# artiom-matvei/RLAO

Measured on AMD Instinct MI355X. Metric: AO env-steps/sec (batched loops), higher is better.
Workload: dtype f32; 1 GPU; 8m / 20x20 Shack-Hartmann, 256 batched envs per GPU, integrator closed loop (BASELINE.json configs[1]); envs_per_gpu=256, envs_total=256, resolution=120, n_valid_act=357, n_signal=632, layers=1, controller=leaky integrator, gain 0.5, noise=photon, parallelism=env-shards x1, all-gather of episode returns

## Files before the change

rlao_amd/csrc/ring_device.hpp:

```cpp
#pragma once
#include "common.hpp"

namespace ao {

__device__ inline int torus(int r, int c, int oy, int ox, int S) {
    int pr = r + oy, pc = c + ox;
    pr = pr >= S ? pr - S : pr;
    pc = pc >= S ? pc - S : pc;
    return pr * S + pc;
}

template <typename T>
__device__ inline void gather_ring(const T* __restrict__ map, T* __restrict__ zx, const int* __restrict__ inner_idx, int S,
                                   int n_inner, int K, int sx, int sy, int oy, int ox, int e, int t0, int nt) {
    const T* src = map + (size_t)e * S * S;
    for (int k = t0; k < n_inner; k += nt) {
        const int idx = inner_idx[k];
        const int r = idx / S - sy, c = idx % S - sx;
        zx[(size_t)e * K + k] = src[torus(r, c, oy, ox, S)];
    }
}

__device__ inline uint32_t mt_temper(uint32_t y) {
    y ^= (y >> 11);
    y ^= (y << 7) & 0x9d2c5680u;
    y ^= (y << 15) & 0xefc60000u;
    y ^= (y >> 18);
    return y;
}

__device__ inline uint32_t mt_mix(uint32_t a, uint32_t b, uint32_t far) {
    uint32_t y = (a & 0x80000000u) | (b & 0x7fffffffu);
    return far ^ (y >> 1) ^ ((y & 1u) ? 0x9908b0dfu : 0u);
}

__device__ inline void mt_twist(uint32_t* s) {
    const int t = threadIdx.x;
    uint32_t v = 0;
    if (t < 227) v = mt_mix(s[t], s[t + 1], s[t + 397]);
    __syncthreads();
    if (t < 227) s[t] = v;
    __syncthreads();
    if (t < 227) v = mt_mix(s[t + 227], s[t + 228], s[t]);
    __syncthreads();
    if (t < 227) s[t + 227] = v;
    __syncthreads();
    if (t < 169) v = mt_mix(s[t + 454], s[t + 455], s[t + 227]);
    __syncthreads();
    if (t < 169) s[t + 454] = v;
    __syncthreads();
    if (t == 0) s[623] = mt_mix(s[623], s[0], s[396]);
    __syncthreads();
}

template <typename T>
__device__ inline void mt_normal_body(const uint32_t* mt_state, const int* mt_pos, uint32_t* mt_state_out, int* mt_pos_out,
                                      T* __restrict__ zx, int K, int n_inner, int n_outer, int e, const double* xi_scale) {
    __shared__ uint32_t s[kMtN];
    __shared__ int scan[256];
    __shared__ int sh_pos, sh_got, sh_stop;
    const int t = threadIdx.x;
    const uint32_t* gs = mt_state + (size_t)e * kMtN;
    uint32_t* gso = mt_state_out + (size_t)e * kMtN;
    for (int i = t; i < kMtN; i += 256) s[i] = gs[i];
    if (t == 0) {
        sh_pos = mt_pos[e];
        sh_got = 0;
    }
    __syncthreads();
    const int need_pairs = n_outer / 2;
    T* out = zx + (size_t)e * K + n_inner;
    while (true) {
        if (sh_pos >= kMtN) {
            mt_twist(s);
            if (t == 0) sh_pos = 0;
            __syncthreads();
        }
        const int pos = sh_pos, got = sh_got;
        const int avail = (kMtN - pos) / 4;
        int acc = 0;
        double n0 = 0.0, n1 = 0.0;
        if (t < avail) {
            const uint32_t* w = s + pos + 4 * t;
            const double d1 = ((double)(mt_temper(w[0]) >> 5) * 67108864.0 + (double)(mt_temper(w[1]) >> 6)) /
                              9007199254740992.0;
            const double d2 = ((double)(mt_temper(w[2]) >> 5) * 67108864.0 + (double)(mt_temper(w[3]) >> 6)) /
                              9007199254740992.0;
            const double x1 = 2.0 * d1 - 1.0, x2 = 2.0 * d2 - 1.0;
            const double r2 = x1 * x1 + x2 * x2;
            if (r2 < 1.0 && r2 != 0.0) {
                acc = 1;
                const double f = sqrt(-2.0 * log(r2) / r2);
                n0 = f * x2;
                n1 = f * x1;
                if (xi_scale) {
                    const double sg = xi_scale[e];
                    n0 *= sg;
                    n1 *= sg;
                }
            }
        }
        const unsigned long long bal = __ballot(acc);
        const int lane = t & (kWave - 1), wv = t / kWave;
        const int in_wave = __popcll(bal & ((lane == 63) ? ~0ull : ((2ull << lane) - 1ull)));
        if (lane == 0) scan[wv] = __popcll(bal);
        __syncthreads();
        int before = 0;
        for (int q = 0; q < wv; ++q) before += scan[q];
        const int total_acc = scan[0] + scan[1] + scan[2] + scan[3];
        const int incl = before + in_wave;
        const int remaining = need_pairs - got;
        if (t == 0) sh_stop = -1;
        __syncthreads();
        if (acc && incl <= remaining) {
            const int j = got + incl - 1;
            out[2 * j] = (T)n0;
            out[2 * j + 1] = (T)n1;
            if (incl == remaining) sh_stop = t;
        }
        __syncthreads();
        if (sh_stop >= 0) {
            if (t == 0) sh_pos = pos + 4 * (sh_stop + 1);
            break;
        }
        if (t == 0) {
            sh_pos = kMtN;
            sh_got = got + total_acc;
        }
        __syncthreads();
    }
    __syncthreads();
    for (int i = t; i < kMtN; i += 256) gso[i] = s[i];
    if (t == 0) mt_pos_out[e] = sh_pos;
}

}
```

Measured before the change: 5.653 million env-steps/s.

## Batch multiple Mersenne Twister twists per round and process two polar pairs per thread

```diff
diff --git a/rlao_amd/csrc/ring_device.hpp b/rlao_amd/csrc/ring_device.hpp
--- a/rlao_amd/csrc/ring_device.hpp
+++ b/rlao_amd/csrc/ring_device.hpp
@@ -34,104 +34,116 @@
     return far ^ (y >> 1) ^ ((y & 1u) ? 0x9908b0dfu : 0u);
 }
 
-__device__ inline void mt_twist(uint32_t* s) {
+constexpr int kMtTry = kMtN / 4;
+constexpr int kMtSlots = 4;
+constexpr int kMtLaneTry = 2 * 256;
+
+__device__ inline void mt_twist_next(const uint32_t* s, uint32_t* n) {
     const int t = threadIdx.x;
-    uint32_t v = 0;
-    if (t < 227) v = mt_mix(s[t], s[t + 1], s[t + 397]);
+    if (t < 227) n[t] = mt_mix(s[t], s[t + 1], s[t + 397]);
     __syncthreads();
-    if (t < 227) s[t] = v;
+    if (t < 227) n[t + 227] = mt_mix(s[t + 227], s[t + 228], n[t]);
     __syncthreads();
-    if (t < 227) v = mt_mix(s[t + 227], s[t + 228], s[t]);
+    if (t < 169) n[t + 454] = mt_mix(s[t + 454], s[t + 455], n[t + 227]);
+    if (t == 192) n[623] = mt_mix(s[623], n[0], n[396]);
     __syncthreads();
-    if (t < 227) s[t + 227] = v;
-    __syncthreads();
-    if (t < 169) v = mt_mix(s[t + 454], s[t + 455], s[t + 227]);
-    __syncthreads();
-    if (t < 169) s[t + 454] = v;
-    __syncthreads();
-    if (t == 0) s[623] = mt_mix(s[623], s[0], s[396]);
-    __syncthreads();
+}
+
+__device__ inline bool mt_polar(const uint32_t* w, double& n0, double& n1) {
+#pragma clang fp contract(off)
+    const double d1 = ((double)(mt_temper(w[0]) >> 5) * 67108864.0 + (double)(mt_temper(w[1]) >> 6)) /
+                      9007199254740992.0;
+    const double d2 = ((double)(mt_temper(w[2]) >> 5) * 67108864.0 + (double)(mt_temper(w[3]) >> 6)) /
+                      9007199254740992.0;
+    const double x1 = 2.0 * d1 - 1.0, x2 = 2.0 * d2 - 1.0;
+    const double r2 = x1 * x1 + x2 * x2;
+    if (!(r2 < 1.0 && r2 != 0.0)) return false;
+    const double f = sqrt(-2.0 * log(r2) / r2);
+    n0 = f * x2;
+    n1 = f * x1;
+    return true;
 }
 
 template <typename T>
 __device__ inline void mt_normal_body(const uint32_t* mt_state, const int* mt_pos, uint32_t* mt_state_out, int* mt_pos_out,
                                       T* __restrict__ zx, int K, int n_inner, int n_outer, int e, const double* xi_scale) {
-    __shared__ uint32_t s[kMtN];
-    __shared__ int scan[256];
-    __shared__ int sh_pos, sh_got, sh_stop;
+    __shared__ uint32_t s[kMtSlots * kMtN];
+    __shared__ int scan[4];
+    __shared__ int sh_stop;
     const int t = threadIdx.x;
+    const int lane = t & (kWave - 1), wv = t / kWave;
     const uint32_t* gs = mt_state + (size_t)e * kMtN;
     uint32_t* gso = mt_state_out + (size_t)e * kMtN;
     for (int i = t; i < kMtN; i += 256) s[i] = gs[i];
-    if (t == 0) {
-        sh_pos = mt_pos[e];
-        sh_got = 0;
-    }
+    int pos = mt_pos[e], got = 0, cur = 0;
+    const double sg = xi_scale ? xi_scale[e] : 1.0;
     __syncthreads();
     const int need_pairs = n_outer / 2;
     T* out = zx + (size_t)e * K + n_inner;
-    while (true) {
-        if (sh_pos >= kMtN) {
-            mt_twist(s);
-            if (t == 0) sh_pos = 0;
-            __syncthreads();
-        }
-        const int pos = sh_pos, got = sh_got;
-        const int avail = (kMtN - pos) / 4;
-        int acc = 0;
-        double n0 = 0.0, n1 = 0.0;
-        if (t < avail) {
-            const uint32_t* w = s + pos + 4 * t;
-            const double d1 = ((double)(mt_temper(w[0]) >> 5) * 67108864.0 + (double)(mt_temper(w[1]) >> 6)) /
-                              9007199254740992.0;
-            const double d2 = ((double)(mt_temper(w[2]) >> 5) * 67108864.0 + (double)(mt_temper(w[3]) >> 6)) /
-                              9007199254740992.0;
-            const double x1 = 2.0 * d1 - 1.0, x2 = 2.0 * d2 - 1.0;
-            const double r2 = x1 * x1 + x2 * x2;
-            if (r2 < 1.0 && r2 != 0.0) {
-                acc = 1;
-                const double f = sqrt(-2.0 * log(r2) / r2);
-                n0 = f * x2;
-                n1 = f * x1;
-                if (xi_scale) {
-                    const double sg = xi_scale[e];
-                    n0 *= sg;
-                    n1 *= sg;
+    auto slot = [](int b) { return b >= kMtSlots ? b - kMtSlots : b; };
+    while (got < need_pairs) {
+        const int remaining = need_pairs - got;
+        const int avail0 = (kMtN - pos) / 4;
+        const int want = remaining + remaining / 3 + 16 - avail0;
+        const int nt = want <= 0 ? 0 : min((kMtLaneTry - avail0) / kMtTry, (want + kMtTry - 1) / kMtTry);
+        for (int j = 0; j < nt; ++j) mt_twist_next(s + slot(cur + j) * kMtN, s + slot(cur + j + 1) * kMtN);
+        const int n_try = avail0 + kMtTry * nt;
+        bool acc[2];
+        double n0[2], n1[2];
+#pragma unroll
+        for (int u = 0; u < 2; ++u) {
+            const int a = 2 * t + u;
+            acc[u] = false;
+            n0[u] = n1[u] = 0.0;
+            if (a < n_try) {
+                const int a2 = a - avail0;
+                const uint32_t* w = a2 < 0 ? s + cur * kMtN + pos + 4 * a
+                                           : s + slot(cur + 1 + a2 / kMtTry) * kMtN + 4 * (a2 % kMtTry);
+                acc[u] = mt_polar(w, n0[u], n1[u]);
+                if (acc[u] && xi_scale) {
+                    n0[u] *= sg;
+                    n1[u] *= sg;
                 }
             }
         }
-        const unsigned long long bal = __ballot(acc);
-        const int lane = t & (kWave - 1), wv = t / kWave;
-        const int in_wave = __popcll(bal & ((lane == 63) ? ~0ull : ((2ull << lane) - 1ull)));
-        if (lane == 0) scan[wv] = __popcll(bal);
+        const unsigned long long bal0 = __ballot(acc[0]), bal1 = __ballot(acc[1]);
+        const unsigned long long below = (1ull << lane) - 1ull;
+        const int in_wave = __popcll(bal0 & below) + __popcll(bal1 & below);
+        if (lane == 0) scan[wv] = __popcll(bal0) + __popcll(bal1);
+        if (t == 0) sh_stop = -1;
         __syncthreads();
-        int before = 0;
+        int before = in_wave;
         for (int q = 0; q < wv; ++q) before += scan[q];
         const int total_acc = scan[0] + scan[1] + scan[2] + scan[3];
-        const int incl = before + in_wave;
-        const int remaining = need_pairs - got;
-        if (t == 0) sh_stop = -1;
-        __syncthreads();
-        if (acc && incl <= remaining) {
-            const int j = got + incl - 1;
-            out[2 * j] = (T)n0;
-            out[2 * j + 1] = (T)n1;
-            if (incl == remaining) sh_stop = t;
+#pragma unroll
+        for (int u = 0; u < 2; ++u) {
+            before += acc[u] ? 1 : 0;
+            if (acc[u] && before <= remaining) {
+                const int j = got + before - 1;
+                out[2 * j] = (T)n0[u];
+                out[2 * j + 1] = (T)n1[u];
+                if (before == remaining) sh_stop = 2 * t + u;
+            }
         }
         __syncthreads();
-        if (sh_stop >= 0) {
-            if (t == 0) sh_pos = pos + 4 * (sh_stop + 1);
-            break;
-        }
-        if (t == 0) {
-            sh_pos = kMtN;
-            sh_got = got + total_acc;
+        const int stop = sh_stop;
+        if (stop >= 0) {
+            const int a2 = stop - avail0;
+            if (a2 < 0) pos += 4 * (stop + 1);
+            else {
+                cur = slot(cur + 1 + a2 / kMtTry);
+                pos = 4 * (a2 % kMtTry + 1);
+            }
+            got = need_pairs;
+        } else {
+            cur = slot(cur + nt);
+            pos = kMtN;
+            got += total_acc;
         }
         __syncthreads();
     }
-    __syncthreads();
-    for (int i = t; i < kMtN; i += 256) gso[i] = s[i];
-    if (t == 0) mt_pos_out[e] = sh_pos;
+    for (int i = t; i < kMtN; i += 256) gso[i] = s[cur * kMtN + i];
+    if (t == 0) mt_pos_out[e] = pos;
 }
 
 }
```

Result: faster. 5.726 million env-steps/s, median of 6 (+1.3%).
